# kaisun24/CPU-Vision

Hardware: AMD Instinct MI355X
Metric: Mpixels/sec on 3x3 conv2d, 4K fp32 frames (higher is better)
Workload: dtype f32

## Files before the change

cpu-vision_amd/csrc/conv3x3_c3.hip:

```cpp
#include <cstdlib>

#include "mv_common.h"
#include "mv_act.h"

namespace mv {

typedef float f32x16 __attribute__((ext_vector_type(16)));
typedef float f32x4 __attribute__((ext_vector_type(4)));


struct C3Args {
  const float* x;
  const float* w;
  const float* b;
  float* y;
  int cout, h, wdt;
  int mtiles;
  int th;
  int wc;
  int pitch;
  int tiles_x, tiles_y;
  int groups;
  int relu;
  int vec_rows;
  unsigned nblocks;
  float mean[3], stdv[3];
};

constexpr int kKS = 14;
constexpr int kK = 27;

__device__ constexpr int c3_row(int k) { return k / 3; }
__device__ constexpr int c3_dx(int k) { return k % 3; }

template <bool RELU>
__device__ inline float c3_act(float v) {
  if (RELU) v = relu_f32(v);
  return v;
}

template <bool RELU, bool FULL, bool FULLM, bool IN_U8>
__global__ __launch_bounds__(256, 2) void k_conv3x3_c3(const C3Args A) {
  extern __shared__ __attribute__((aligned(16))) float lds[];
  const int tid = threadIdx.x, lane = tid & (kWave - 1);
  const int wave = __builtin_amdgcn_readfirstlane(tid >> 6);
  const int l31 = lane & 31, hf = lane >> 5;
  const int cout = A.cout, h = A.h, w = A.wdt;
  const int th = A.th, wc = A.wc, pitch = A.pitch;
  const int tile_rows = th + 2;
  float* xin = lds;
  float* wfr = lds + 3 * tile_rows * pitch + 16;

  const unsigned wid = xcd_remap(blockIdx.x, A.nblocks);
  const int tx = wid % A.tiles_x;
  const unsigned t2 = wid / A.tiles_x;
  const int ty = t2 % A.tiles_y;
  const long long img = t2 / A.tiles_y;
  const int xb = tx * wc, yb = ty * th;
  const float* xp = A.x + (size_t)img * 3 * h * w;
  const uint8_t* xpu = reinterpret_cast<const uint8_t*>(A.x) + (size_t)img * 3 * h * w;
  const size_t plane = (size_t)h * w;
  auto norm = [&](unsigned byte, int ci) -> float {
    const float v = (float)byte * (float)(1.0 / 255.0);
    return (v - A.mean[ci]) / A.stdv[ci];
  };

  for (int q = wave; q < A.mtiles * kKS; q += 4) {
    const int s = q % kKS, m = q / kKS;
    const int co = 32 * m + l31, k = 2 * s + hf;
    float v = 0.f;
    if (co < cout && k < kK) v = A.w[(size_t)co * kK + k];
    if (co < cout && k == kK && A.b != nullptr) v = A.b[co];
    wfr[q * 64 + lane] = v;
  }
  {
    constexpr int kStage = 8;
    const int cols = wc + 2;
    const int rows_total = 3 * tile_rows;
    if (A.vec_rows) {
      const int nq = (wc + 8) >> 2;
      const int per_row = (nq + kWave - 1) / kWave;
      const int nitems = rows_total * per_row;
      for (int base = wave; base < nitems; base += 4 * kStage) {
        f32x4 v[kStage];
#pragma unroll
        for (int u = 0; u < kStage; ++u) {
          const int it = base + 4 * u;
          v[u] = (f32x4){0.f, 0.f, 0.f, 0.f};
          if (it < nitems) {
            const int r = it / per_row, q = (it - r * per_row) * kWave + lane;
            const int ci = r / tile_rows, rr = r - ci * tile_rows;
            const int gy = yb - 1 + rr, gx0 = xb - 4 + 4 * q;
            if (q < nq && gy >= 0 && gy < h && gx0 >= 0 && gx0 + 3 < w) {
              if constexpr (IN_U8) {
                const unsigned b4 = *reinterpret_cast<const unsigned*>(xpu + ((size_t)ci * h + gy) * w + gx0);
                v[u] = (f32x4){norm(b4 & 0xffu, ci), norm((b4 >> 8) & 0xffu, ci), norm((b4 >> 16) & 0xffu, ci), norm(b4 >> 24, ci)};
              } else {
                v[u] = *reinterpret_cast<const f32x4*>(xp + ((size_t)ci * h + gy) * w + gx0);
              }
            }
          }
        }
#pragma unroll
        for (int u = 0; u < kStage; ++u) {
          const int it = base + 4 * u;
          if (it < nitems) {
            const int r = it / per_row, q = (it - r * per_row) * kWave + lane;
            if (q < nq) {
              float* dst = xin + r * pitch + (4 * q - 3);
              const float e[4] = {v[u].x, v[u].y, v[u].z, v[u].w};
#pragma unroll
              for (int j = 0; j < 4; ++j) {
                const int c = 4 * q - 3 + j;
                if (c >= 0 && c < cols) dst[j] = e[j];
              }
            }
          }
        }
      }
    } else {
      const int per_row = (cols + kWave - 1) / kWave;
      const int nitems = rows_total * per_row;
      for (int base = wave; base < nitems; base += 4 * kStage) {
        float v[kStage];
#pragma unroll
        for (int u = 0; u < kStage; ++u) {
          const int it = base + 4 * u;
          v[u] = 0.f;
          if (it < nitems) {
            const int r = it / per_row, c = (it - r * per_row) * kWave + lane;
            const int ci = r / tile_rows, rr = r - ci * tile_rows;
            const int gy = yb - 1 + rr, gx = xb - 1 + c;
            if (c < cols && gy >= 0 && gy < h && gx >= 0 && gx < w) {
              if constexpr (IN_U8)
                v[u] = norm(xpu[((size_t)ci * h + gy) * w + gx], ci);
              else
                v[u] = xp[((size_t)ci * h + gy) * w + gx];
            }
          }
        }
#pragma unroll
        for (int u = 0; u < kStage; ++u) {
          const int it = base + 4 * u;
          if (it < nitems) {
            const int r = it / per_row, c = (it - r * per_row) * kWave + lane;
            if (c < cols) xin[r * pitch + c] = v[u];
          }
        }
      }
    }
  }
  __syncthreads();

  const int m = (A.mtiles == 2) ? (wave >> 1) : 0;
  const int gfirst = (A.mtiles == 2) ? (wave & 1) : wave;
  const int gstep = (A.mtiles == 2) ? 2 : 4;
  const int ng = (A.groups > gfirst) ? (A.groups - gfirst + gstep - 1) / gstep : 0;
  if (ng == 0) return;

  float afr[kKS];
#pragma unroll
  for (int s = 0; s < kKS; ++s) afr[s] = wfr[(m * kKS + s) * 64 + lane];

  int rowoff[9];
#pragma unroll
  for (int r = 0; r < 9; ++r) rowoff[r] = ((r / 3) * tile_rows + (r % 3)) * pitch;

  char* const simg = reinterpret_cast<char*>(A.y + (size_t)img * cout * plane);
  const unsigned chan_off = (unsigned)((size_t)(32 * m + 4 * hf) * plane * sizeof(float));

  auto geom = [&](int j, int& lbase, unsigned& voff, bool& ok) {
    const int g = gfirst + gstep * j;
    const unsigned f = 128u * (unsigned)g + 4u * (unsigned)l31;
    const unsigned ly = f / (unsigned)wc, lx = f - ly * (unsigned)wc;
    lbase = (int)(ly * (unsigned)pitch + lx);
    const int gy = yb + (int)ly, gx = xb + (int)lx;
    ok = FULL || (gy < h && gx < w && (int)ly < th);
    voff = chan_off + (unsigned)(((size_t)gy * w + gx) * sizeof(float));
  };
  auto load_row = [&](f32x4 (&dst)[2], int lbase, int r) {
    const float* p = xin + lbase + rowoff[r];
    dst[0] = *reinterpret_cast<const f32x4*>(p);
    dst[1] = *reinterpret_cast<const f32x4*>(p + 4);
  };
  auto elem = [](const f32x4 (&q)[2], int i) -> float {
    const f32x4& v = q[i >> 2];
    return (i & 3) == 0 ? v.x : (i & 3) == 1 ? v.y : (i & 3) == 2 ? v.z : v.w;
  };
  auto drain = [&](const f32x16 (&acc)[4], int i, unsigned voff, bool ok) {
    const int cu = (i & 3) + 8 * (i >> 2);
    f32x4 v = {c3_act<RELU>(acc[0][i]), c3_act<RELU>(acc[1][i]), c3_act<RELU>(acc[2][i]), c3_act<RELU>(acc[3][i])};
    f32x4* dst = reinterpret_cast<f32x4*>(simg + (size_t)cu * plane * sizeof(float) + voff);
    if ((FULL || ok) && (FULLM || 32 * m + cu + 4 * hf < cout)) *dst = v;
  };
  const f32x16 zero = {0.f, 0.f, 0.f, 0.f, 0.f, 0.f, 0.f, 0.f, 0.f, 0.f, 0.f, 0.f, 0.f, 0.f, 0.f, 0.f};

  f32x16 accA[4], accB[4];
  f32x4 row[9][2];
  f32x4 nrow[2][2];
  int lb_cur, lb_next;
  unsigned vo_cur, vo_prev = 0;
  bool ok_cur, ok_prev = false;
  geom(0, lb_cur, vo_cur, ok_cur);
  load_row(nrow[0], lb_cur, 0);
  load_row(nrow[1], lb_cur, 1);

#define MV_C3_GROUP(cur, prev, j, have_prev)                                                             \
  {                                                                                                      \
    unsigned vo_n = 0;                                                                                   \
    bool ok_n = false;                                                                                   \
    geom(min((j) + 1, ng - 1), lb_next, vo_n, ok_n);                                                      \
    row[0][0] = nrow[0][0], row[0][1] = nrow[0][1], row[1][0] = nrow[1][0], row[1][1] = nrow[1][1];       \
    _Pragma("unroll") for (int s = 0; s < kKS; ++s) {                                                    \
                    \
      constexpr_for_rows(s)                                                                              \
      _Pragma("unroll") for (int a = 0; a < 4; ++a) {                                                    \
        const int k0 = 2 * s, k1 = 2 * s + 1;                                                            \
        const float b0 = elem(row[c3_row(k0)], a + c3_dx(k0));                                           \
        const float b1 = (k1 < kK) ? elem(row[c3_row(k1 < kK ? k1 : 0)], a + c3_dx(k1)) : 1.0f;           \
        const float bsel = hf ? b1 : b0;                                                                 \
        cur[a] = __builtin_amdgcn_mfma_f32_32x32x2f32(afr[s], bsel, s == 0 ? zero : cur[a], 0, 0, 0);      \
        if (have_prev) {                                                                                 \
          const int slot = 4 * s + a;                                                                    \
          if (slot % 3 == 2 && slot / 3 < 16) drain(prev, slot / 3, vo_prev, ok_prev);                    \
        }                                                                                                \
      }                                                                                                  \
      if (s == 10) load_row(nrow[0], lb_next, 0);                                                        \
      if (s == 12) load_row(nrow[1], lb_next, 1);                                                        \
    }                                                                                                    \
    vo_prev = vo_cur, ok_prev = ok_cur;                                                                  \
    lb_cur = lb_next, vo_cur = vo_n, ok_cur = ok_n;                                                      \
  }
#define constexpr_for_rows(s)                                                                            \
  _Pragma("unroll") for (int r = 2; r < 9; ++r) {                                                        \
    if ((3 * r) / 2 - 1 == (s)) load_row(row[r], lb_cur, r);                                             \
  }

  MV_C3_GROUP(accA, accB, 0, false)
  int j = 1;
  for (; j + 1 < ng; j += 2) {
    MV_C3_GROUP(accB, accA, j, true)
    MV_C3_GROUP(accA, accB, j + 1, true)
  }
  if (j < ng) {
    MV_C3_GROUP(accB, accA, j, true)
#pragma unroll
    for (int i = 0; i < 16; ++i) drain(accB, i, vo_prev, ok_prev);
  } else {
#pragma unroll
    for (int i = 0; i < 16; ++i) drain(accA, i, vo_prev, ok_prev);
  }
#undef MV_C3_GROUP
#undef constexpr_for_rows
}

template <bool RELU, bool FULL, bool FULLM, bool IN_U8>
static int c3_launch_t(const C3Args& a, size_t lds_bytes, hipStream_t s) {
  auto k = k_conv3x3_c3<RELU, FULL, FULLM, IN_U8>;
  if (lds_bytes > 48 * 1024)
    (void)hipFuncSetAttribute(reinterpret_cast<const void*>(k), hipFuncAttributeMaxDynamicSharedMemorySize, (int)lds_bytes);
  hipLaunchKernelGGL(k, dim3(a.nblocks), dim3(256), lds_bytes, s, a);
  return check_launch("k_conv3x3_c3");
}

template <bool RELU, bool FULL, bool FULLM>
static int c3_launch(const C3Args& a, size_t lds_bytes, bool in_u8, hipStream_t s) {
  return in_u8 ? c3_launch_t<RELU, FULL, FULLM, true>(a, lds_bytes, s) : c3_launch_t<RELU, FULL, FULLM, false>(a, lds_bytes, s);
}

bool conv3x3_c3_supported(const float* x, const float* y, int cin, int cout, int h, int w) {
  const char* v = tune_env("MV_FORCE_GENERIC_CONV");
  if (v && *v && *v != '0') return false;
  if (cin != 3 || cout > 64 || cout < 1) return false;
  if (w % 4 != 0 || (uintptr_t)y % 16 != 0) return false;
  if ((size_t)cout * h * w * sizeof(float) >= (1ull << 32)) return false;
  (void)x;
  return true;
}

int launch_conv3x3_c3(const void* xv, bool in_u8, const float* mean3, const float* std3, const float* w, const float* b,
                      float* y, int64_t n, int h, int wdt, int cout, int relu, hipStream_t s) {
  C3Args a = {};
  const float* x = static_cast<const float*>(xv);
  a.x = x, a.w = w, a.b = b, a.y = y;
  for (int i = 0; i < 3; ++i) a.mean[i] = in_u8 ? mean3[i] : 0.f, a.stdv[i] = in_u8 ? std3[i] : 1.f;
  a.cout = cout, a.h = h, a.wdt = wdt, a.relu = relu;
  a.mtiles = (cout + 31) / 32;
  a.vec_rows = (wdt % 4 == 0) && ((uintptr_t)x % (in_u8 ? 4 : 16) == 0);
  const bool flat = wdt <= 256;
  a.wc = flat ? wdt : 256;
  a.pitch = ((a.wc + 2 + 3) & ~3) + 8;
  int th = 16;
  if (const char* e = tune_env("MV_C3_TH")) th = atoi(e) > 0 ? atoi(e) : th;
  auto bytes = [&](int rows) {
    return ((size_t)3 * (rows + 2) * a.pitch + 16 + (size_t)a.mtiles * kKS * 64) * sizeof(float);
  };
  while (th > 1 && bytes(th) > 150 * 1024) th >>= 1;
  if (!tune_env("MV_C3_TH"))
    while (th > 4 && (long long)n * ((wdt + a.wc - 1) / a.wc) * ((h + th - 1) / th) < 512) th >>= 1;
  if (th > h) th = h;
  a.th = th;
  a.tiles_x = (wdt + a.wc - 1) / a.wc;
  a.tiles_y = (h + th - 1) / th;
  a.groups = (th * a.wc + 127) / 128;
  const long long nb = (long long)n * a.tiles_x * a.tiles_y;
  if (nb > 0x7fffffffLL) return set_error(MV_ERR_UNSUPPORTED, "conv3x3: batch too large for one launch");
  a.nblocks = (unsigned)nb;
  const size_t lds_bytes = bytes(th);
  const bool full = (h % th == 0) && (wdt % a.wc == 0) && ((th * a.wc) % 128 == 0);
  const bool fullm = (cout % 32 == 0);
#define MV_C3_DISPATCH(R)                                                               \
  if (full && fullm) return c3_launch<R, true, true>(a, lds_bytes, in_u8, s);             \
  if (full) return c3_launch<R, true, false>(a, lds_bytes, in_u8, s);                     \
  if (fullm) return c3_launch<R, false, true>(a, lds_bytes, in_u8, s);                    \
  return c3_launch<R, false, false>(a, lds_bytes, in_u8, s);
  if (relu) {
    MV_C3_DISPATCH(true)
  }
  MV_C3_DISPATCH(false)
#undef MV_C3_DISPATCH
}

}
```

Measured before the change: 260,000.

## Load conv weights directly into registers, drop LDS weight staging, deepen input staging

Each lane now loads its weight and bias fragment straight from global memory into registers instead of staging all weights through LDS and reading them back after the barrier. This frees the weight region of LDS, which can allow larger tiles or more occupancy. The input staging batch grows from 8 to 14 in-flight quad loads. Row/channel index math is also simplified with a per_row==1 fast path and compare-based channel index. The change costs more registers and issues redundant global weight loads per block.

New measurement: 259,900. No clear change (-0.0%).

```diff
diff --git a/cpu-vision_amd/csrc/conv3x3_c3.hip b/cpu-vision_amd/csrc/conv3x3_c3.hip
--- a/cpu-vision_amd/csrc/conv3x3_c3.hip
+++ b/cpu-vision_amd/csrc/conv3x3_c3.hip
@@ -49,7 +49,6 @@
   const int th = A.th, wc = A.wc, pitch = A.pitch;
   const int tile_rows = th + 2;
   float* xin = lds;
-  float* wfr = lds + 3 * tile_rows * pitch + 16;
 
   const unsigned wid = xcd_remap(blockIdx.x, A.nblocks);
   const int tx = wid % A.tiles_x;
@@ -65,31 +64,38 @@
     return (v - A.mean[ci]) / A.stdv[ci];
   };
 
-  for (int q = wave; q < A.mtiles * kKS; q += 4) {
-    const int s = q % kKS, m = q / kKS;
-    const int co = 32 * m + l31, k = 2 * s + hf;
-    float v = 0.f;
-    if (co < cout && k < kK) v = A.w[(size_t)co * kK + k];
-    if (co < cout && k == kK && A.b != nullptr) v = A.b[co];
-    wfr[q * 64 + lane] = v;
-  }
+  const int m = (A.mtiles == 2) ? (wave >> 1) : 0;
+  const int gfirst = (A.mtiles == 2) ? (wave & 1) : wave;
+  const int gstep = (A.mtiles == 2) ? 2 : 4;
+  const int ng = (A.groups > gfirst) ? (A.groups - gfirst + gstep - 1) / gstep : 0;
+
+  float afr[kKS];
+  float bias_raw = 0.f;
+  const bool afr_live = 32 * m + l31 < cout;
   {
-    constexpr int kStage = 8;
+    const int co = afr_live ? 32 * m + l31 : cout - 1;
+#pragma unroll
+    for (int s = 0; s < kKS; ++s) afr[s] = A.w[(size_t)co * kK + (2 * s + hf < kK ? 2 * s + hf : kK - 1)];
+    if (A.b != nullptr) bias_raw = A.b[co];
+  }
+  {
+    constexpr int kStage = 14;
     const int cols = wc + 2;
     const int rows_total = 3 * tile_rows;
     if (A.vec_rows) {
       const int nq = (wc + 8) >> 2;
       const int per_row = (nq + kWave - 1) / kWave;
       const int nitems = rows_total * per_row;
-      for (int base = wave; base < nitems; base += 4 * kStage) {
+      const bool one_quad = per_row == 1;
+      auto stage_quads = [&](int base) {
         f32x4 v[kStage];
 #pragma unroll
         for (int u = 0; u < kStage; ++u) {
           const int it = base + 4 * u;
           v[u] = (f32x4){0.f, 0.f, 0.f, 0.f};
           if (it < nitems) {
-            const int r = it / per_row, q = (it - r * per_row) * kWave + lane;
-            const int ci = r / tile_rows, rr = r - ci * tile_rows;
+            const int r = one_quad ? it : it / per_row, q = (it - r * per_row) * kWave + lane;
+            const int ci = (r >= tile_rows) + (r >= 2 * tile_rows), rr = r - ci * tile_rows;
             const int gy = yb - 1 + rr, gx0 = xb - 4 + 4 * q;
             if (q < nq && gy >= 0 && gy < h && gx0 >= 0 && gx0 + 3 < w) {
               if constexpr (IN_U8) {
@@ -105,7 +111,7 @@
         for (int u = 0; u < kStage; ++u) {
           const int it = base + 4 * u;
           if (it < nitems) {
-            const int r = it / per_row, q = (it - r * per_row) * kWave + lane;
+            const int r = one_quad ? it : it / per_row, q = (it - r * per_row) * kWave + lane;
             if (q < nq) {
               float* dst = xin + r * pitch + (4 * q - 3);
               const float e[4] = {v[u].x, v[u].y, v[u].z, v[u].w};
@@ -117,7 +123,9 @@
             }
           }
         }
-      }
+      };
+      stage_quads(wave);
+      for (int base = wave + 4 * kStage; base < nitems; base += 4 * kStage) stage_quads(base);
     } else {
       const int per_row = (cols + kWave - 1) / kWave;
       const int nitems = rows_total * per_row;
@@ -151,16 +159,10 @@
     }
   }
   __syncthreads();
-
-  const int m = (A.mtiles == 2) ? (wave >> 1) : 0;
-  const int gfirst = (A.mtiles == 2) ? (wave & 1) : wave;
-  const int gstep = (A.mtiles == 2) ? 2 : 4;
-  const int ng = (A.groups > gfirst) ? (A.groups - gfirst + gstep - 1) / gstep : 0;
   if (ng == 0) return;
-
-  float afr[kKS];
-#pragma unroll
-  for (int s = 0; s < kKS; ++s) afr[s] = wfr[(m * kKS + s) * 64 + lane];
+#pragma unroll
+  for (int s = 0; s < kKS; ++s) afr[s] = afr_live ? afr[s] : 0.f;
+  if (hf) afr[kKS - 1] = afr_live ? bias_raw : 0.f;
 
   int rowoff[9];
 #pragma unroll
@@ -293,7 +295,7 @@
   int th = 16;
   if (const char* e = tune_env("MV_C3_TH")) th = atoi(e) > 0 ? atoi(e) : th;
   auto bytes = [&](int rows) {
-    return ((size_t)3 * (rows + 2) * a.pitch + 16 + (size_t)a.mtiles * kKS * 64) * sizeof(float);
+    return ((size_t)3 * (rows + 2) * a.pitch + 16) * sizeof(float);
   };
   while (th > 1 && bytes(th) > 150 * 1024) th >>= 1;
   if (!tune_env("MV_C3_TH"))
```
